# cgtuebingen/3D-RE-GEN

Measured on AMD Instinct MI355X. Metric: objects/sec (50-step Hunyuan3D-2 DiT + 256^3 marching cubes), higher is better.
Workload: dtype bf16; 1 GPU; configs[1]: 5 synthetic 512x512 RGBA crops per GPU, Hunyuan3D-2 full dims bf16, 50 flow-matching steps x CFG 2, 257^3 grid query + Lewiner marching cubes; weights=seeded synthetic, objects_total=5, objects_per_launch=4, parallelism=object-parallel x1

## Files before the change

3d-re-gen_amd/csrc/gemm.hip:

```cpp
#include <hip/hip_runtime.h>
#include <stdint.h>
#include <string.h>

#include <map>
#include <mutex>
#include <type_traits>
#include <utility>

#include "gemm_common.h"
#include "wave_sum.h"
#include "kernels.h"
#include "prof.h"

namespace r3g {
namespace {

constexpr int BK = 64;

template <int B, int E, int S, typename F>
__device__ __forceinline__ void static_for(F&& f) {
    if constexpr (B < E) {
        f(std::integral_constant<int, B>{});
        static_for<B + S, E, S>(f);
    }
}

template <bool GLDS, int NW, int ROWS>
__device__ __forceinline__ void stage_tile(const uint16_t* __restrict__ src, int64_t ld, int row0, int rows_valid,
                                           int k0, char* lds_tile, int wid, int lane, int tid) {
    if constexpr (GLDS) {
#pragma unroll
        for (int i = 0; i < ROWS / 8 / NW; ++i) {
            const int piece = wid * (ROWS / 8 / NW) + i;
            const int row = piece * 8 + (lane >> 3);
            const int kc = (lane & 7) ^ ((row >> 1) & 7);
            int gr = row0 + row;
            gr = gr < rows_valid ? gr : rows_valid - 1;
            const uint16_t* g = src + (int64_t)gr * ld + k0 + kc * 8;
            __builtin_amdgcn_global_load_lds((const __attribute__((address_space(1))) void*)g,
                                             (__attribute__((address_space(3))) void*)(lds_tile + piece * 1024), 16, 0, 0);
        }
    } else {
        uint4 v[ROWS / 8 / NW];
#pragma unroll
        for (int i = 0; i < ROWS / 8 / NW; ++i) {
            const int c = i * (NW * 64) + tid;
            const int row = c >> 3, kc = c & 7;
            int gr = row0 + row;
            gr = gr < rows_valid ? gr : rows_valid - 1;
            v[i] = *reinterpret_cast<const uint4*>(src + (int64_t)gr * ld + k0 + kc * 8);
        }
#pragma unroll
        for (int i = 0; i < ROWS / 8 / NW; ++i) {
            const int c = i * (NW * 64) + tid;
            const int row = c >> 3, kc = c & 7;
            *reinterpret_cast<uint4*>(lds_tile + row * 128 + ((kc ^ ((row >> 1) & 7)) << 4)) = v[i];
        }
    }
}

#define R3G_LDS __attribute__((address_space(3)))
typedef R3G_LDS char* LdsP;
typedef uint32_t u32x4v __attribute__((ext_vector_type(4)));
typedef uint32_t u32x2v __attribute__((ext_vector_type(2)));
__device__ __forceinline__ uint4 lds_ld4(const R3G_LDS char* a) { const u32x4v v = *reinterpret_cast<const R3G_LDS u32x4v*>(a); return make_uint4(v[0], v[1], v[2], v[3]); }
__device__ __forceinline__ uint2 lds_ld2(const R3G_LDS char* a) { const u32x2v v = *reinterpret_cast<const R3G_LDS u32x2v*>(a); return make_uint2(v[0], v[1]); }
__device__ __forceinline__ void lds_st2(R3G_LDS char* a, uint2 v) { *reinterpret_cast<R3G_LDS u32x2v*>(a) = (u32x2v){v.x, v.y}; }
__device__ __forceinline__ LdsP lds_ptr(char* generic_smem_ptr) { return (LdsP)generic_smem_ptr; }

template <int EPI, int MI, bool SMALLREG, int PI = MI, bool VM0 = false, int SLICE = 2048>
__device__ __forceinline__ void gemm_epilogue(const GemmArgs& p, f32x4 (&acc)[4][MI], int m0, int n0, int batch, int wr,
                                              int wc, int lane, LdsP lds_wave = nullptr, bool have_lds = false,
                                              const f32x4* bias_pre = nullptr) {
    constexpr int WROWS = MI * 16;
    static_assert(MI % PI == 0, "scratch passes");
    static_assert(SLICE == 2048 || ((EPI == EPI_QKV || EPI == EPI_BF16 || EPI == EPI_BF16_GELU_TANH || EPI == EPI_BF16_GELU_ERF || EPI == EPI_BF16_GELU_ERF_LNF) && PI == 4),
                  "sliced scratch: 64-row passes of 128-byte rows");
    auto roff = [](int R) __attribute__((always_inline)) { return SLICE == 2048 ? R * 128 : (R >> 4) * SLICE + (R & 15) * 128; };
    if constexpr (EPI == EPI_QKV) {
        const QkvEpi& e = p.qkv;
        const int g = (n0 + wc * 64) >> 6;
        if (n0 + wc * 64 >= p.N) {
            if (VM0) asm volatile("s_waitcnt vmcnt(0)" ::: "memory");
            return;
        }
        int type, head;
        if (e.layout == QKV_KHD) { type = g / e.heads; head = g - type * e.heads; }
        else if (e.layout == QKV_HEAD_QKV) { head = g / 3; type = g - head * 3; }
        else if (e.layout == QKV_HEAD_KV) { head = g >> 1; type = 1 + (g & 1); }
        else { type = 0; head = g; }
        const int dbase = (lane >> 4) << 2;
        int sg_n = e.nseg, sg_m0[3], sg_m1[3], sg_b[3], sg_d[3];
#pragma unroll
        for (int sgi = 0; sgi < 3; ++sgi) { sg_m0[sgi] = e.seg_m0[sgi]; sg_m1[sgi] = e.seg_m1[sgi]; sg_b[sgi] = e.seg_batch[sgi]; sg_d[sgi] = e.seg_dst[sgi]; }
        if (e.nseg > 3) {
            const int mw_u = __builtin_amdgcn_readfirstlane(m0 + wr * WROWS);
            const int4* tab = reinterpret_cast<const int4*>(e.seg_tab);
            int4 t = make_int4(0, 0, 0, 0);
            if (lane < e.nseg) t = tab[lane];
            const int first = __popcll(__ballot(lane < e.nseg && t.y <= mw_u));
            sg_n = 3;
#pragma unroll
            for (int sgi = 0; sgi < 3; ++sgi) {
                const int idx = first + sgi;
                const bool ok = idx < e.nseg;
                const int li = ok ? idx : 0;
                sg_m0[sgi] = ok ? __builtin_amdgcn_readlane(t.x, li) : 0;
                sg_m1[sgi] = ok ? __builtin_amdgcn_readlane(t.y, li) : 0;
                sg_b[sgi] = __builtin_amdgcn_readlane(t.z, li);
                sg_d[sgi] = __builtin_amdgcn_readlane(t.w, li);
            }
        }
        const float* nw = type == 0 ? e.qw : e.kw;
        const float* nb = type == 0 ? e.qb : e.kb;
        const bool do_norm = type < 2 && e.norm != QKN_NONE;
        f32x4 bias4[4], nw4[4], nb4[4];
#pragma unroll
        for (int j = 0; j < 4; ++j) {
            bias4[j] = (f32x4){0.f, 0.f, 0.f, 0.f};
            nw4[j] = (f32x4){1.f, 1.f, 1.f, 1.f};
            nb4[j] = (f32x4){0.f, 0.f, 0.f, 0.f};
            if (p.bias) bias4[j] = *reinterpret_cast<const f32x4*>(p.bias + n0 + wc * 64 + j * 16 + dbase);
            if (do_norm && nw) nw4[j] = *reinterpret_cast<const f32x4*>(nw + j * 16 + dbase);
            if (do_norm && e.norm == QKN_LAYERNORM && nb) nb4[j] = *reinterpret_cast<const f32x4*>(nb + j * 16 + dbase);
        }
        constexpr int PROWS = PI * 16;
        auto flush_pass = [&](const int ip) __attribute__((always_inline)) {
            __builtin_amdgcn_fence(__ATOMIC_ACQ_REL, "wavefront");
            __builtin_amdgcn_wave_barrier();
            if (VM0 && ip == 0) asm volatile("s_waitcnt vmcnt(0)" ::: "memory");
            auto map_row = [&](int m, int& ob, int64_t& drow) {
                ob = batch;
                drow = (int64_t)e.dst_row0 + m;
                if (m >= p.M) return false;
                if (sg_n == 0) return true;
                bool hit = false;
#pragma unroll
                for (int sgi = 0; sgi < 3; ++sgi)
                    if (sgi < sg_n && m >= sg_m0[sgi] && m < sg_m1[sgi]) {
                        hit = true;
                        ob = sg_b[sgi];
                        drow = (int64_t)sg_d[sgi] + (m - sg_m0[sgi]);
                    }
                return hit;
            };
            const int mw = m0 + wr * WROWS + ip * 16;
            const int mw_u = __builtin_amdgcn_readfirstlane(mw);
            bool whole = mw_u + PROWS <= p.M;
            int w_ob = batch;
            int64_t w_drow = (int64_t)e.dst_row0 + mw_u;
            if (sg_n > 0) {
                bool hit = false;
#pragma unroll
                for (int sgi = 0; sgi < 3; ++sgi)
                    if (sgi < sg_n && mw_u >= sg_m0[sgi] && mw_u + PROWS <= sg_m1[sgi]) {
                        hit = true;
                        w_ob = sg_b[sgi];
                        w_drow = (int64_t)sg_d[sgi] + (mw_u - sg_m0[sgi]);
                    }
                whole = whole && hit;
// ... 165 lines not shown
            }
            if (type < 2) {
                uint16_t* base = (type == 0 ? e.Q + (((int64_t)ob * e.heads + head) * e.Lq_pad + drow) * 64
                                            : e.K + (((int64_t)ob * e.heads + head) * e.Lk_pad + drow) * 64);
#pragma unroll
                for (int j = 0; j < 4; ++j) {
                    uint2 pk;
                    pk.x = pack_bf16(v[j][0], v[j][1]);
                    pk.y = pack_bf16(v[j][2], v[j][3]);
                    *reinterpret_cast<uint2*>(base + j * 16 + dbase) = pk;
                }
            } else {
                uint16_t* base = e.Vt + (((int64_t)ob * e.heads + head) * 64) * (int64_t)e.Lk_pad + vt_key_pos(drow);
#pragma unroll
                for (int j = 0; j < 4; ++j)
#pragma unroll
                    for (int c = 0; c < 4; ++c)
                        base[(int64_t)(j * 16 + dbase + c) * e.Lk_pad] = (uint16_t)(pack_bf16(v[j][c], 0.f) & 0xFFFFu);
            }
        }
        if constexpr (kWide) flush_pass(ip);
        });
        };
        if (have_lds) all_passes(std::true_type{});
        else all_passes(std::false_type{});
        return;
    }
    const int mrow = m0 + wr * WROWS + (lane & 15);
    const int ncol = n0 + wc * 64 + ((lane >> 4) << 2);
    const float* gate = p.gate ? p.gate + (int64_t)batch * p.strideGate : nullptr;
    if constexpr (EPI == EPI_FP8_GELU_ERF) {
        uint8_t* C8 = reinterpret_cast<uint8_t*>(p.C) + (int64_t)batch * p.strideC;
        const float inv = p.out_inv_scale;
        const bool wide = have_lds && PI == MI && (p.N & 15) == 0 && (p.ldc & 15) == 0 && (p.strideC & 15) == 0 &&
                          (reinterpret_cast<uintptr_t>(p.C) & 15) == 0;
#pragma unroll
        for (int j = 0; j < 4; ++j) {
            const int n = ncol + j * 16;
            f32x4 bj = (f32x4){0.f, 0.f, 0.f, 0.f};
            if (p.bias) bj = *reinterpret_cast<const f32x4*>(p.bias + (n < p.N ? n : p.N - 4));
#pragma unroll
            for (int i = 0; i < MI; ++i) {
                f32x4 v = gelu_erf4<false>(acc[j][i] + bj) * inv;
#pragma unroll
                for (int c = 0; c < 4; ++c) v[c] = __builtin_fabsf(v[c]) > 448.f ? __builtin_copysignf(448.f, v[c]) : v[c];
                int w = 0;
                w = __builtin_amdgcn_cvt_pk_fp8_f32(v[0], v[1], w, false);
                w = __builtin_amdgcn_cvt_pk_fp8_f32(v[2], v[3], w, true);
                const int r = i * 16 + (lane & 15), m = mrow + i * 16;
                if (wide) *reinterpret_cast<R3G_LDS uint32_t*>(lds_wave + r * 64 + ((j ^ (r & 3)) << 4) + ((lane >> 4) << 2)) = (uint32_t)w;
                else if (n < p.N && m < p.M) *reinterpret_cast<uint32_t*>(C8 + (int64_t)m * p.ldc + n) = (uint32_t)w;
            }
        }
        if (wide) {
            __builtin_amdgcn_fence(__ATOMIC_ACQ_REL, "wavefront");
            __builtin_amdgcn_wave_barrier();
            const int cc = lane & 3, n = n0 + wc * 64 + cc * 16;
#pragma unroll
            for (int t = 0; t < WROWS / 16; ++t) {
                const int rr = t * 16 + (lane >> 2);
                const int m = m0 + wr * WROWS + rr;
                const uint4 d = lds_ld4(lds_wave + rr * 64 + ((cc ^ (rr & 3)) << 4));
                if (m < p.M && n < p.N) *reinterpret_cast<uint4*>(C8 + (int64_t)m * p.ldc + n) = d;
            }
        }
        return;
    }
    if constexpr (EPI == EPI_RESID_BF16 || EPI == EPI_RESID_F16 || EPI == EPI_RESID_BF16_LND || EPI == EPI_RESID_BF16_ST) {
        constexpr bool F16 = EPI == EPI_RESID_F16;
        constexpr bool ST = EPI == EPI_RESID_BF16_ST;
        constexpr bool LND = EPI == EPI_RESID_BF16_LND || ST;
        uint16_t* X = reinterpret_cast<uint16_t*>(p.C) + (int64_t)batch * p.strideC;
        const uint16_t* XR = p.resid_src ? p.resid_src + (int64_t)batch * p.strideC : X;
        f32x4 bj[4], gj[4];
#pragma unroll
        for (int j = 0; j < 4; ++j) {
            const int nb = ncol + j * 16;
            const int nbc = nb < p.N ? nb : p.N - 4;
            bj[j] = (f32x4){0.f, 0.f, 0.f, 0.f};
            gj[j] = (f32x4){1.f, 1.f, 1.f, 1.f};
            if (p.bias) bj[j] = *reinterpret_cast<const f32x4*>(p.bias + nbc);
            if (gate) gj[j] = *reinterpret_cast<const f32x4*>(gate + nbc);
        }
        const bool wide = have_lds && PI >= 2 && (p.N & 7) == 0 && (p.ldc & 7) == 0 && (p.strideC & 7) == 0 &&
                          (reinterpret_cast<uintptr_t>(p.C) & 15) == 0 && (reinterpret_cast<uintptr_t>(XR) & 15) == 0;
        if (wide) {
            constexpr int RP = PI * 8;
            constexpr int GP = PI / 2;
            const int cc = lane & 7;
            const int n = n0 + wc * 64 + cc * 8;
            f32x4 gw0 = (f32x4){0.f, 0.f, 0.f, 0.f}, gw1 = gw0;
            if constexpr (LND && !ST) {
                const int nc = n < p.N ? n : p.N - 8;
                gw0 = *reinterpret_cast<const f32x4*>(p.lnd_gw + nc);
                gw1 = *reinterpret_cast<const f32x4*>(p.lnd_gw + nc + 4);
            }
            const bool full = m0 + wr * WROWS + WROWS <= p.M && n0 + wc * 64 + 64 <= p.N;
            const int64_t row0 = (int64_t)(m0 + wr * WROWS + (lane >> 3)) * p.ldc + n, step8 = 8 * (int64_t)p.ldc;
#pragma unroll
            for (int ip = 0; ip < MI; ip += GP) {
                uint4 old[RP / 8];
                if (full) {
#pragma unroll
                    for (int t = 0; t < RP / 8; ++t)
                        old[t] = *reinterpret_cast<const uint4*>(XR + row0 + (int64_t)(ip * 2 + t) * step8);
                } else {
#pragma unroll
                    for (int t = 0; t < RP / 8; ++t) {
                        const int m = m0 + wr * WROWS + ip * 16 + t * 8 + (lane >> 3);
                        const int mc = m < p.M ? m : p.M - 1;
                        const int nc = n < p.N ? n : p.N - 8;
                        old[t] = *reinterpret_cast<const uint4*>(XR + (int64_t)mc * p.ldc + nc);
                    }
                }
#pragma unroll
                for (int j = 0; j < 4; ++j)
#pragma unroll
                    for (int ii = 0; ii < GP; ++ii) {
                        const int r = ii * 16 + (lane & 15);
                        const int chunk = (j * 4 + (lane >> 4)) ^ (r & 15);
                        *reinterpret_cast<R3G_LDS f32x4*>(lds_wave + r * 256 + chunk * 16) = gj[j] * (acc[j][ip + ii] + bj[j]);
                    }
                __builtin_amdgcn_fence(__ATOMIC_ACQ_REL, "wavefront");
                __builtin_amdgcn_wave_barrier();
                auto rows_out = [&](auto FULLC) __attribute__((always_inline)) {
                constexpr bool kFull = decltype(FULLC)::value;
#pragma unroll
                for (int t = 0; t < RP / 8; ++t) {
                    const int rr = t * 8 + (lane >> 3);
                    const int m = m0 + wr * WROWS + ip * 16 + rr;
                    const f32x4 d0 = *reinterpret_cast<const R3G_LDS f32x4*>(lds_wave + rr * 256 + (((2 * cc) ^ (rr & 15)) << 4));
                    const f32x4 d1 = *reinterpret_cast<const R3G_LDS f32x4*>(lds_wave + rr * 256 + (((2 * cc + 1) ^ (rr & 15)) << 4));
                    const uint32_t o[4] = {old[t].x, old[t].y, old[t].z, old[t].w};
                    uint32_t q[4];
#pragma unroll
                    for (int k = 0; k < 4; ++k) {
                        const f32x2 ov = unpack16<F16>(o[k]);
                        const f32x4& d = k < 2 ? d0 : d1;
                        q[k] = pack16<F16>(ov[0] + d[(k & 1) * 2], ov[1] + d[(k & 1) * 2 + 1]);
                    }
                    if constexpr (LND) {
                        float v[8];
#pragma unroll
                        for (int k = 0; k < 4; ++k) {
                            const f32x2 u = unpack16<false>(q[k]);
                            v[2 * k] = u[0];
                            v[2 * k + 1] = u[1];
                        }
                        float s1 = ((v[0] + v[1]) + (v[2] + v[3])) + ((v[4] + v[5]) + (v[6] + v[7]));
                        s1 += lane_xor<1>(s1);
                        s1 += lane_xor<2>(s1);
                        s1 += lane_xor<4>(s1);
                        const float mu = s1 * (1.0f / 64.0f);
                        float m2 = 0.f, s3 = 0.f;
#pragma unroll
                        for (int k = 0; k < 8; ++k) {
                            const float dv = v[k] - mu;
                            m2 = fmaf(dv, dv, m2);
                            s3 = fmaf(v[k], k < 4 ? gw0[k] : gw1[k - 4], s3);
                        }
                        m2 += lane_xor<1>(m2); s3 += lane_xor<1>(s3);
                        m2 += lane_xor<2>(m2); s3 += lane_xor<2>(s3);
                        m2 += lane_xor<4>(m2); s3 += lane_xor<4>(s3);
                        if (cc == 0 && m < p.M && n < p.N)
                            *reinterpret_cast<f32x4*>(p.lnd_part + ((int64_t)m * (p.N >> 6) + ((n0 >> 6) + wc)) * 4) = (f32x4){s1, m2, s3, 0.f};
                    }
                    if constexpr (!LND || ST) {
                        if constexpr (kFull) *reinterpret_cast<uint4*>(X + row0 + (int64_t)(ip * 2 + t) * step8) = make_uint4(q[0], q[1], q[2], q[3]);
                        else if (m < p.M && n < p.N) *reinterpret_cast<uint4*>(X + (int64_t)m * p.ldc + n) = make_uint4(q[0], q[1], q[2], q[3]);
                    }
                }
                };
                if (full) rows_out(std::true_type{});
                else rows_out(std::false_type{});
                __builtin_amdgcn_fence(__ATOMIC_ACQ_REL, "wavefront");
                __builtin_amdgcn_wave_barrier();
            }
            return;
        }
        if constexpr (LND) return;
#pragma unroll
        for (int j = 0; j < 4; ++j) {
            uint2 old[MI];
#pragma unroll
            for (int i = 0; i < MI; ++i) {
                const int n = ncol + j * 16, m = mrow + i * 16;
                const int nc = n < p.N ? n : p.N - 4, mc = m < p.M ? m : p.M - 1;
                old[i] = *reinterpret_cast<const uint2*>(XR + (int64_t)mc * p.ldc + nc);
            }
#pragma unroll
            for (int i = 0; i < MI; ++i) {
                const int n = ncol + j * 16, m = mrow + i * 16;
                const f32x4 d = gj[j] * (acc[j][i] + bj[j]);
                uint2 pk;
                const f32x2 ox = unpack16<F16>(old[i].x), oy = unpack16<F16>(old[i].y);
                pk.x = pack16<F16>(ox[0] + d[0], ox[1] + d[1]);
                pk.y = pack16<F16>(oy[0] + d[2], oy[1] + d[3]);
                if (n < p.N && m < p.M) *reinterpret_cast<uint2*>(X + (int64_t)m * p.ldc + n) = pk;
            }
        }
        return;
    }
    if constexpr (EPI == EPI_RESID_F32) {
        float* X = reinterpret_cast<float*>(p.C) + (int64_t)batch * p.strideC;
        const bool wide = have_lds && (p.ldc & 3) == 0 && (p.strideC & 3) == 0 &&
                          (reinterpret_cast<uintptr_t>(p.C) & 15) == 0;
        if (wide) {
            const int cc = lane & 7;
#pragma unroll
            for (int jp = 0; jp < 2; ++jp) {
                f32x4 bj[2], gj[2];
#pragma unroll
                for (int jj = 0; jj < 2; ++jj) {
                    const int nb = ncol + (2 * jp + jj) * 16;
                    const int nbc = nb < p.N ? nb : p.N - 4;
                    bj[jj] = (f32x4){0.f, 0.f, 0.f, 0.f};
                    gj[jj] = (f32x4){1.f, 1.f, 1.f, 1.f};
                    if (p.bias) bj[jj] = *reinterpret_cast<const f32x4*>(p.bias + nbc);
                    if (gate) gj[jj] = *reinterpret_cast<const f32x4*>(gate + nbc);
                }
                const int n = n0 + wc * 64 + jp * 32 + cc * 4;
                const int nc = n < p.N ? n : p.N - 4;
#pragma unroll
                for (int ip = 0; ip < MI; ip += PI) {
#pragma unroll
                    for (int jj = 0; jj < 2; ++jj)
#pragma unroll
                        for (int ii = 0; ii < PI; ++ii) {
                            const int r = ii * 16 + (lane & 15);
                            const int chunk = (jj * 4 + (lane >> 4)) ^ (r & 7);
                            *reinterpret_cast<R3G_LDS f32x4*>(lds_wave + r * 128 + chunk * 16) = gj[jj] * (acc[2 * jp + jj][ip + ii] + bj[jj]);
                        }
                    __builtin_amdgcn_fence(__ATOMIC_ACQ_REL, "wavefront");
                    __builtin_amdgcn_wave_barrier();
                    if (VM0 && jp == 0 && ip == 0) asm volatile("s_waitcnt vmcnt(0)" ::: "memory");
#pragma unroll
                    for (int t0 = 0; t0 < PI * 2; t0 += 4) {
                        f32x4 old[4];
#pragma unroll
                        for (int tt = 0; tt < 4; ++tt) {
                            const int m = m0 + wr * WROWS + ip * 16 + (t0 + tt) * 8 + (lane >> 3);
                            const int mc = m < p.M ? m : p.M - 1;
                            old[tt] = *reinterpret_cast<const f32x4*>(X + (int64_t)mc * p.ldc + nc);
                        }
#pragma unroll
                        for (int tt = 0; tt < 4; ++tt) {
                            const int rr = (t0 + tt) * 8 + (lane >> 3);
                            const int m = m0 + wr * WROWS + ip * 16 + rr;
                            const f32x4 d = *reinterpret_cast<const R3G_LDS f32x4*>(lds_wave + rr * 128 + ((cc ^ (rr & 7)) << 4));
                            if (n < p.N && m < p.M) *reinterpret_cast<f32x4*>(X + (int64_t)m * p.ldc + n) = old[tt] + d;
                        }
                    }
                    __builtin_amdgcn_fence(__ATOMIC_ACQ_REL, "wavefront");
// ... 1109 lines not shown
        R3G_SB();
        R3G_BAR();
        read_a(1, b);
        R3G_SB();
        if (!last) stage_a(0, t + 2, b);
        R3G_BAR();
        R3G_SB();
        mma(I1{}, I1{});
        R3G_SB();
        R3G_BAR();
        if (!last) {
            stage_w(1, t + 2, b);
            asm volatile("s_waitcnt vmcnt(6)" ::: "memory");
        } else if (b == 0) {
            asm volatile("s_waitcnt vmcnt(0)" ::: "memory");
        }
        R3G_BAR();
        R3G_SB();
        mma(I1{}, I0{});
        R3G_SB();
        R3G_BAR();
    };
    using T = std::true_type;
    using F = std::false_type;

    auto locate_u = [&](int index, Tile& tl, int& nk) {
        tl = locate(index);
        tl.second = __builtin_amdgcn_readfirstlane(tl.second);
        tl.batch = __builtin_amdgcn_readfirstlane(tl.batch);
        tl.m0 = __builtin_amdgcn_readfirstlane(tl.m0);
        tl.n0 = __builtin_amdgcn_readfirstlane(tl.n0);
        nk = args_of(tl.second).K / BK;
    };
    Tile cur;
    int nk;
    int my = wg_first;
    locate_u(my, cur, nk);
    set_sources(cur);
    stage_w(0, 0, 0); stage_a(0, 0, 0); stage_w(1, 0, 0); stage_a(1, 0, 0);
    R3G_STAMP_DECL;
    for (;;) {
        R3G_STAMP(5);
        stage_w(0, 1, 1); stage_a(0, 1, 1); stage_w(1, 1, 1);
        __builtin_amdgcn_s_waitcnt(0x0F76);
        R3G_BAR();
        if (wr == 1) R3G_BAR();
        R3G_STAMP(0);
        int t = 0;
        for (; t + 2 < nk; t += 2) {
            four_phases(I0{}, F{}, t);
            four_phases(I1{}, F{}, t + 1);
        }
        four_phases(I0{}, T{}, t);
        four_phases(I1{}, T{}, t + 1);
        if (wr == 0) R3G_BAR();
        R3G_STAMP(1);

        const Tile done = cur;
        int lane_e = lane;
        asm volatile("" : "+v"(lane_e));
        f32x4 bias_pre[4];
        {
            const GemmArgs& pp = args_of(done.second);
#pragma unroll
            for (int j = 0; j < 4; ++j) {
                const int n = done.n0 + wc * 64 + ((lane_e >> 4) << 2) + j * 16;
                bias_pre[j] = (f32x4){0.f, 0.f, 0.f, 0.f};
                if (pp.bias) bias_pre[j] = *reinterpret_cast<const f32x4*>(pp.bias + (n < pp.N ? n : pp.N - 4));
            }
        }
        my += xcd_wgs;
        const bool more = my < xcd_end;
        if (more) {
            locate_u(my, cur, nk);
            set_sources(cur);
            stage_w(0, 0, 0); stage_a(0, 0, 0); stage_w(1, 0, 0); stage_a(1, 0, 0);
        }
        R3G_STAMP(2);
        {
            const GemmArgs& pp = args_of(done.second);
            auto run = [&](auto E) __attribute__((always_inline)) {
                constexpr int epi = decltype(E)::value;
                constexpr bool kPre = epi == EPI_BF16 || epi == EPI_BF16_GELU_TANH || epi == EPI_BF16_GELU_ERF || epi == EPI_BF16_GELU_ERF_LNF;
                constexpr bool kSl = SLICED && (kPre || epi == EPI_QKV);
                if constexpr (kSl)
                    gemm_epilogue<epi, MI, true, 4, false, HALF>(pp, acc, done.m0, done.n0, done.batch, wr, wc, lane_e,
                                                                 lds_ptr(smem + BUF + wid * 2048), true, kPre ? bias_pre : nullptr);
                else
                    gemm_epilogue<epi, MI, true, 2, false>(pp, acc, done.m0, done.n0, done.batch, wr, wc, lane_e,
                                                           lds_ptr(smem + 2 * BUF + wid * 4096), pp.wide_epilogue != 0, kPre ? bias_pre : nullptr);
            };
            if constexpr (EPI2 != EPI) {
                if (done.second) run(std::integral_constant<int, EPI2>{});
                else run(std::integral_constant<int, EPI>{});
            } else {
                run(std::integral_constant<int, EPI>{});
            }
        }
        R3G_STAMP(3);
        if (!more) break;
        asm volatile("" : "+s"(cur.m0), "+s"(cur.n0), "+s"(cur.batch));
        set_sources(cur);
#pragma unroll
        for (int j = 0; j < 4; ++j)
#pragma unroll
            for (int i = 0; i < MI; ++i) acc[j][i] = (f32x4){0.f, 0.f, 0.f, 0.f};
    }
    R3G_STAMP_OUT;
}

#ifdef R3G_GEMM_STAMPS
}
}
extern "C" __attribute__((visibility("default"))) int r3g_debug_gemm_stamps(unsigned long long* out64) {
    return (int)hipMemcpyFromSymbol(out64, HIP_SYMBOL(r3g::g_gemm_stamps), sizeof(unsigned long long) * 64);
}
namespace r3g {
namespace {
#endif

int g_gemm_xcd_walk = 1;
int g_gemm_persistent_qkv = 1;
int g_gemm_epi_slices = 1;
int g_gemm_mixed = 1;

template <int EPI, int EPI2 = EPI>
hipError_t launch_gemm8p(const GemmArgs& p, const GemmArgs& p2, int num_cu, hipStream_t s) {
    int tiles = ((p.N + 255) / 256) * ((p.M + 255) / 256) * p.batch;
    if (p2.M > 0) tiles += ((p2.N + 255) / 256) * ((p2.M + 255) / 256) * p2.batch;
    const int rounds = (tiles + num_cu - 1) / num_cu;
    const int grid = (tiles + rounds - 1) / rounds;
    const size_t lds = 163840;
    constexpr bool kSliceable = EPI == EPI_BF16 || EPI == EPI_BF16_GELU_TANH || EPI == EPI_BF16_GELU_ERF || EPI == EPI_QKV || EPI == EPI_BF16_GELU_ERF_LNF;
    auto k = gemm8p_kernel<EPI, false, EPI2>;
    auto ks = gemm8p_kernel<EPI, kSliceable, EPI2>;
    static int state = 0;
    if (state == 0) {
        state = hipFuncSetAttribute((const void*)k, hipFuncAttributeMaxDynamicSharedMemorySize, (int)lds) == hipSuccess ? 1 : -1;
        if (state > 0 && kSliceable)
            state = hipFuncSetAttribute((const void*)ks, hipFuncAttributeMaxDynamicSharedMemorySize, (int)lds) == hipSuccess ? 1 : -1;
    }
    if (state < 0) { (void)hipGetLastError(); return hipErrorNotSupported; }
    const int walk = g_gemm_xcd_walk ? rounds : 0;
    counter_add(EPI2 != EPI ? LC_GEMM_MIXED : LC_GEMM_PHASED_PERSISTENT);
    if (kSliceable && g_gemm_epi_slices && p.wide_epilogue) { hipLaunchKernelGGL(ks, dim3(grid), dim3(512), lds, s, p, p2, tiles, walk); }
    else { hipLaunchKernelGGL(k, dim3(grid), dim3(512), lds, s, p, p2, tiles, walk); }
    return hipGetLastError();
}

template <int EPI>
hipError_t launch_gemm8(const GemmArgs& p, const GemmArgs& p2, hipStream_t s) {
    int tiles = ((p.N + 255) / 256) * ((p.M + 255) / 256) * p.batch;
    if (p2.M > 0) tiles += ((p2.N + 255) / 256) * ((p2.M + 255) / 256) * p2.batch;
    const size_t lds = 131072;
    auto k = gemm8_kernel<EPI, false>;
    static bool done = false;
    if (!done) {
        done = true;
        (void)hipFuncSetAttribute((const void*)k, hipFuncAttributeMaxDynamicSharedMemorySize, (int)lds);
    }
    counter_add(LC_GEMM_PHASED);
    hipLaunchKernelGGL(k, dim3(tiles), dim3(512), lds, s, p, p2, (float*)nullptr, (unsigned*)nullptr, 0u);
    return hipGetLastError();
}

constexpr int kSplitMaxTiles = 128;
struct SplitWs { float* ws = nullptr; unsigned* flags = nullptr; unsigned epoch = 0; };
static std::mutex g_split_mutex;
static std::map<std::pair<int, hipStream_t>, SplitWs> g_split;

template <int EPI>
hipError_t launch_gemm8_split(const GemmArgs& p, const GemmArgs& p2, hipStream_t s) {
    int tiles = ((p.N + 255) / 256) * ((p.M + 255) / 256) * p.batch;
    if (p2.M > 0) tiles += ((p2.N + 255) / 256) * ((p2.M + 255) / 256) * p2.batch;
    if (tiles > kSplitMaxTiles) return hipErrorNotSupported;
    int dev = 0;
    hipError_t e = hipGetDevice(&dev);
    if (e != hipSuccess) return e;
    SplitWs w;
    {
        std::lock_guard<std::mutex> lock(g_split_mutex);
        SplitWs& slot = g_split[std::make_pair(dev, s)];
        if (!slot.ws) {
            e = hipMalloc((void**)&slot.ws, (size_t)kSplitMaxTiles * 256 * 256 * 4);
            if (e != hipSuccess) return e;
            e = hipMalloc((void**)&slot.flags, (size_t)kSplitMaxTiles * 8 * 4);
            if (e != hipSuccess) return e;
            e = hipMemset(slot.flags, 0, (size_t)kSplitMaxTiles * 8 * 4);
            if (e != hipSuccess) return e;
        }
        if (++slot.epoch == 0u) slot.epoch = 1u;
        w = slot;
    }
    const size_t lds = 131072;
    auto k = gemm8_kernel<EPI, true>;
    static bool done = false;
    if (!done) {
        done = true;
        (void)hipFuncSetAttribute((const void*)k, hipFuncAttributeMaxDynamicSharedMemorySize, (int)lds);
    }
    counter_add(LC_GEMM_SPLITK2);
    hipLaunchKernelGGL(k, dim3(2 * tiles), dim3(512), lds, s, p, p2, w.ws, w.flags, w.epoch);
    return hipGetLastError();
}

template <int EPI>
hipError_t launch_deep(const GemmArgs& p, int batch, hipStream_t s) {
    const int tiles = ((p.N + 255) / 256) * ((p.M + 255) / 256) * batch;
    const size_t lds = 4 * 2 * 256 * 32 * 2;
    auto k = gemm_deep_kernel<EPI>;
    static bool done = false;
    if (!done) {
        done = true;
        (void)hipFuncSetAttribute((const void*)k, hipFuncAttributeMaxDynamicSharedMemorySize, (int)lds);
    }
    counter_add(LC_GEMM_DEEP_RING);
// ... 14 lines not shown
        if (!done) {
            done = true;
            (void)hipFuncSetAttribute((const void*)kt, hipFuncAttributeMaxDynamicSharedMemorySize, (int)lds);
            (void)hipFuncSetAttribute((const void*)kf, hipFuncAttributeMaxDynamicSharedMemorySize, (int)lds);
        }
    }
    counter_add(BIG == 2 ? LC_GEMM_256X128 : BIG == 1 ? (NW == 16 ? LC_GEMM_W16_256 : LC_GEMM_TWO_STAGE_256) : (NW == 4 ? LC_GEMM_W4_128 : LC_GEMM_W8_128));
    if (!glds) counter_add(LC_GEMM_REGISTER_STAGED);
    if (glds) {
        hipLaunchKernelGGL(kt, dim3(tiles), dim3(NW * 64), lds, s, p, p2);
    } else {
        hipLaunchKernelGGL(kf, dim3(tiles), dim3(NW * 64), lds, s, p, p2);
    }
    return hipGetLastError();
}

template <bool RESID>
__global__ __launch_bounds__(256) void splitk_reduce_kernel(const float* __restrict__ ws, int S, int64_t MN, int N,
                                                            const float* __restrict__ bias, const float* __restrict__ gate,
                                                            float* __restrict__ C, int64_t ldc) {
    const int64_t i = ((int64_t)blockIdx.x * 256 + threadIdx.x) * 4;
    if (i >= MN) return;
    f32x4 v = *reinterpret_cast<const f32x4*>(ws + i);
    int s = 1;
    for (; s + 4 <= S; s += 4) {
        f32x4 t[4];
#pragma unroll
        for (int k = 0; k < 4; ++k) t[k] = *reinterpret_cast<const f32x4*>(ws + (int64_t)(s + k) * MN + i);
#pragma unroll
        for (int k = 0; k < 4; ++k) v += t[k];
    }
    for (; s < S; ++s) v += *reinterpret_cast<const f32x4*>(ws + (int64_t)s * MN + i);
    const int64_t m = i / N;
    const int n = (int)(i - m * N);
    if (bias) v += *reinterpret_cast<const f32x4*>(bias + n);
    float* dst = C + m * ldc + n;
    if (RESID) {
        if (gate) v = *reinterpret_cast<const f32x4*>(gate + n) * v;
        v = *reinterpret_cast<const f32x4*>(dst) + v;
    }
    *reinterpret_cast<f32x4*>(dst) = v;
}

int g_gemm_splitk128 = 1;
constexpr int kSplit128Slots = 512;
constexpr int kSplit128MinSteps = 8;

static int splitk128_factor(int M, int N, int K, int num_cu) {
    if (K < 2048 || K % 64) return 1;
    const long tiles = (long)((M + 127) / 128) * ((N + 127) / 128);
    const long slots = (long)kSplit128Slots * num_cu / 256;
    if (tiles * 2 > slots) return 1;
    const int nk = K / 64;
    int best = 1;
    for (int S = 2; S <= 64 && S * tiles <= slots && nk / S >= kSplit128MinSteps; ++S)
        if (nk % S == 0) best = S;
    if (best == 2 && K < 4096) best = 1;
    return best;
}

int g_conv_implicit = 1;

template <int EPI>
hipError_t launch_conv(const GemmArgs& p, hipStream_t s) {
    const int tiles = ((p.N + 127) / 128) * ((p.M + 127) / 128) * p.batch;
    const size_t lds = (size_t)2 * (128 + 128) * BK * 2;
    auto k = conv_gemm_kernel<EPI>;
    static bool done = false;
    if (!done) {
        done = true;
        (void)hipFuncSetAttribute((const void*)k, hipFuncAttributeMaxDynamicSharedMemorySize, (int)lds);
    }
    counter_add(LC_GEMM_CONV_IMPLICIT);
    hipLaunchKernelGGL(k, dim3(tiles), dim3(512), lds, s, p);
    return hipGetLastError();
}

int g_gemm_waves = 0;
int g_gemm_raster = -1;
int g_gemm_auto_rule = 2;
int g_num_cu = 256;
int g_gemm_splitk = 0;
int g_gemm_persistent_resid = 0;
int g_gemm_persistent = 1;
int g_gemm_phased = 1;
int g_gemm_wide_epilogue = 1;
int g_gemm_gelu_pk = 1;

template <int EPI>
hipError_t launch_epi(const GemmArgs& p, const GemmArgs& p2, bool glds, hipStream_t s) {
    int waves = g_gemm_waves;
    const int batch = p.batch;
    if (waves == 0) {
        long t256 = (long)((p.N + 255) / 256) * ((p.M + 255) / 256) * batch;
        if (p2.M > 0) t256 += (long)((p2.N + 255) / 256) * ((p2.M + 255) / 256) * p2.batch;
        const long rounds = (t256 + g_num_cu - 1) / g_num_cu;
        const bool fills = t256 * 10 >= rounds * g_num_cu * 9;
        if (g_gemm_auto_rule == 0) {
            if (p2.M == 0 && p.N % 256 == 0 && t256 >= 128 && (p.K >= 2048 || t256 >= 2048)) waves = 9;
            else waves = p.N <= 1024 ? 8 : 4;
        } else {
            const bool wide_enough = p.N >= 4096 || (g_gemm_auto_rule >= 2 && t256 * 100 >= (long)g_num_cu * 85);
            if ((p2.M == 0 || p2.N % 256 == 0) && p.N % 256 == 0 && t256 >= 128 &&
                (p.K >= 2048 || t256 >= 2048 || (wide_enough && fills)))
                waves = g_gemm_phased ? 11 : 9;
            else waves = 8;
        }
    }
    if constexpr (EPI == EPI_RESID_F32 || EPI == EPI_RESID_BF16 || EPI == EPI_RESID_F16 || EPI == EPI_BF16) {
        long tiles = (long)((p.N + 255) / 256) * ((p.M + 255) / 256) * p.batch;
        if (p2.M > 0) tiles += (long)((p2.N + 255) / 256) * ((p2.M + 255) / 256) * p2.batch;
        const bool shape_ok = p.K % 256 == 0 && p.K >= 512 && (p2.M == 0 || p2.K == p.K) && p.N % 256 == 0 &&
                              (p2.M == 0 || p2.N % 256 == 0) && 2 * tiles <= g_num_cu && tiles <= kSplitMaxTiles;
        if (shape_ok && (waves == 13 || (g_gemm_splitk && g_gemm_waves == 0 && EPI == EPI_RESID_F32 && p.K >= 2048 &&
                                         2 * tiles > g_num_cu / 2))) {
            const hipError_t e = launch_gemm8_split<EPI>(p, p2, s);
            if (e != hipErrorNotSupported) return e;
        }
        if (waves == 13) waves = 11;
    }
    if (waves == 13) waves = 11;
    if ((waves == 11 || waves == 12) && p.K % 128 == 0 && (p2.M == 0 || p2.K % 128 == 0)) {
        {
            long tiles = (long)((p.N + 255) / 256) * ((p.M + 255) / 256) * p.batch;
            if (p2.M > 0) tiles += (long)((p2.N + 255) / 256) * ((p2.M + 255) / 256) * p2.batch;
            const bool resid_ok = (EPI != EPI_RESID_F32 || (g_gemm_persistent_resid & 1)) &&
                                  ((EPI != EPI_RESID_BF16 && EPI != EPI_RESID_F16) || (g_gemm_persistent_resid & 2)) &&
                                  (EPI != EPI_QKV || (g_gemm_persistent_qkv && p.wide_epilogue));
            if (p.K >= 256 && (p2.M == 0 || p2.K >= 256) &&
                (waves == 12 || (g_gemm_persistent && g_gemm_waves == 0 && tiles > g_num_cu && resid_ok && EPI != EPI_F32))) {
                const hipError_t e = launch_gemm8p<EPI>(p, p2, g_num_cu, s);
                if (e != hipErrorNotSupported) return e;
            }
        }
        return launch_gemm8<EPI>(p, p2, s);
    }
    if (waves == 11 || waves == 12) waves = g_gemm_waves == 0 ? 9 : 8;
    if (waves == 32 && p.K % 32 == 0 && p2.M == 0) return launch_deep<EPI>(p, batch, s);
    if (waves == 16) return launch_cfg<EPI, 16, 1>(p, p2, glds, s);
    if (waves == 9) return launch_cfg<EPI, 8, 1>(p, p2, glds, s);
    if (waves == 10) return launch_cfg<EPI, 8, 2>(p, p2, glds, s);
    if (waves == 8) return launch_cfg<EPI, 8, 0>(p, p2, glds, s);
    return launch_cfg<EPI, 4, 0>(p, p2, glds, s);
}

}

int g_gemm_glds = 1;

const Option g_gemm_options[] = {
    {"gemm_waves", &g_gemm_waves, OPT_KEEP,
     [](int v) { return v == 0 || v == 4 || v == 8 || v == 9 || v == 10 || v == 11 || v == 12 || v == 13 || v == 16 || v == 32; }},
    {"gemm_raster", &g_gemm_raster, OPT_ANY},
    {"gemm_auto_rule", &g_gemm_auto_rule, OPT_KEEP, [](int v) { return v >= 0; }},
    {"gemm_num_cu", &g_num_cu, OPT_KEEP, [](int v) { return v > 0; }},
    {"gemm_wide_epilogue", &g_gemm_wide_epilogue},
    {"gemm_phased", &g_gemm_phased},
    {"gemm_persistent", &g_gemm_persistent},
    {"gemm_persistent_resid", &g_gemm_persistent_resid, OPT_MASK, nullptr, 3},
    {"gemm_splitk", &g_gemm_splitk},
    {"gemm_splitk128", &g_gemm_splitk128},
    {"conv_implicit", &g_conv_implicit},
    {"gemm_xcd_walk", &g_gemm_xcd_walk},
    {"gemm_epi_slices", &g_gemm_epi_slices},
    {"gemm_mixed", &g_gemm_mixed},
    {"gemm_persistent_qkv", &g_gemm_persistent_qkv},
    {"gelu_pk", &g_gemm_gelu_pk},
    {}};

bool gemm_conv_implicit() { return g_conv_implicit && g_gemm_glds && g_gemm_waves == 0; }
bool gemm_auto_takes_256(int M, int N, int K) {
    if (g_gemm_waves != 0 || g_gemm_auto_rule == 0) return false;
    const long t256 = (long)((N + 255) / 256) * ((M + 255) / 256);
    const long rounds = (t256 + g_num_cu - 1) / g_num_cu;
    const bool fills = t256 * 10 >= rounds * g_num_cu * 9;
    const bool wide_enough = N >= 4096 || (g_gemm_auto_rule >= 2 && t256 * 100 >= (long)g_num_cu * 85);
    return N % 256 == 0 && t256 >= 128 && (K >= 2048 || t256 >= 2048 || (wide_enough && fills));
}
int gemm_splitk128_factor(int M, int N, int K) { return splitk128_factor(M, N, K, g_num_cu); }

bool gemm_fold_supported(int epi, int M, int N, int K) {
    if (epi != EPI_RESID_BF16_ST && epi != EPI_BF16_GELU_ERF_LNF && epi != EPI_RESID_BF16_LND) return false;
    if (!g_gemm_glds || !g_gemm_wide_epilogue) return false;
    return M > 0 && N > 0 && K % 128 == 0 && K >= 256 && N % 256 == 0;
}

static bool gemm_args_ok(const GemmArgs& p) {
    if (p.epi == EPI_QKV && p.qkv.nseg > 3) {
        if (p.qkv.nseg > 64) return false;
        const int* t = p.qkv.seg_tab_host;
        if (!t || !p.qkv.seg_tab) return false;
        for (int i = 0; i < p.qkv.nseg; ++i) {
            if (t[4 * i] > t[4 * i + 1]) return false;
            if (i > 0 && t[4 * i] < t[4 * (i - 1) + 1]) return false;
            if (i >= 3 && t[4 * i] - t[4 * (i - 3) + 1] + 1 < 128) return false;
        }
    }
    return !(p.K % 64 != 0 || p.K <= 0 || (p.N & 3) || (p.lda & 7) || (p.ldw & 7) || (p.epi == EPI_QKV && p.N % 64));
}

static int g_last_splitk_slices = 1;
int gemm_last_splitk_slices() { return g_last_splitk_slices; }

hipError_t gemm_launch2(const GemmArgs& p_in, int batch, const GemmArgs* p2_in, int batch2, hipStream_t s) {
    GemmArgs p = p_in, p2{};
    g_last_splitk_slices = 1;
    p.batch = batch;
    p.raster_group = g_gemm_raster;
    p.wide_epilogue = g_gemm_wide_epilogue ? 1 : 0;
    p.gelu_pk = g_gemm_gelu_pk ? 1 : 0;
    if (p2_in && p2_in->M > 0 && p2_in->N > 0 && batch2 > 0) {
        p2 = *p2_in;
        p2.batch = batch2;
        p2.raster_group = p.raster_group;
        p2.wide_epilogue = p.wide_epilogue;
        p2.gelu_pk = p.gelu_pk;
        if (p2.epi != p.epi || !gemm_args_ok(p2)) return hipErrorInvalidValue;
    }
    if (p.M <= 0 || p.N <= 0 || batch <= 0) {
        if (p2.M > 0) return gemm_launch2(*p2_in, batch2, nullptr, 0, s);
        return hipSuccess;
    }
    if (!gemm_args_ok(p)) return hipErrorInvalidValue;
    auto alg_bytes = [](const GemmArgs& g) {
        if (g.M <= 0) return 0.0;
        const double out = g.epi == EPI_RESID_F32 ? 8.0 : (g.epi == EPI_F32 || g.epi == EPI_RESID_BF16 || g.epi == EPI_RESID_F16 ? 4.0 : g.epi == EPI_RESID_BF16_LND ? 2.0 : (g.epi == EPI_FP8_GELU_ERF ? 1.0 : 2.0));
        return (double)g.batch * (2.0 * g.M * g.K + out * (double)g.M * g.N) + 2.0 * (double)g.N * g.K;
    };
    ProfScope ps(PC_GEMM, 2.0 * (double)p.M * p.N * p.K * batch + 2.0 * (double)p2.M * p2.N * p2.K * p2.batch, s,
                 alg_bytes(p) + alg_bytes(p2));
    if (p.conv.x) {
        const ConvA& cv = p.conv;
        if (p2.M > 0 || batch != 1 || (p.epi != EPI_F32 && p.epi != EPI_RESID_F32) || !g_gemm_glds || cv.Cin < 64 || cv.Cin % 64 ||
            p.K != 9 * cv.Cin || !cv.zero || cv.Ho < 1 || cv.Wo < 1 || p.M % (cv.Ho * cv.Wo) || (p.ldc & 3) ||
            (reinterpret_cast<uintptr_t>(p.C) & 15))
            return hipErrorInvalidValue;
        const int64_t MN = (int64_t)p.M * p.N;
        int S = 1;
        if (p.split_ws && g_gemm_splitk128) {
            S = splitk128_factor(p.M, p.N, p.K, g_num_cu);
            if ((int64_t)S * MN > p.split_ws_elems) S = 1;
        }
        if (S > 1) {
            g_last_splitk_slices = S;
            counter_add(LC_GEMM_SPLITK128);
            GemmArgs q = p;
            q.K = p.K / S;
            q.batch = S;
            q.strideW = q.K;
            q.bias = nullptr;
            q.gate = nullptr;
            q.C = p.split_ws;
            q.ldc = p.N;
            q.strideC = MN;
            q.epi = EPI_F32;
            q.split_ws = nullptr;
            const hipError_t e = launch_conv<EPI_F32>(q, s);
            if (e != hipSuccess) return e;
            const unsigned blocks = (unsigned)((MN / 4 + 255) / 256);
            if (p.epi == EPI_RESID_F32)
                hipLaunchKernelGGL(splitk_reduce_kernel<true>, dim3(blocks), dim3(256), 0, s, (const float*)p.split_ws, S, MN, p.N,
                                   p.bias, p.gate, reinterpret_cast<float*>(p.C), p.ldc);
            else
                hipLaunchKernelGGL(splitk_reduce_kernel<false>, dim3(blocks), dim3(256), 0, s, (const float*)p.split_ws, S, MN, p.N,
                                   p.bias, p.gate, reinterpret_cast<float*>(p.C), p.ldc);
            return hipGetLastError();
        }
        return p.epi == EPI_F32 ? launch_conv<EPI_F32>(p, s) : launch_conv<EPI_RESID_F32>(p, s);
    }
    if (p.split_ws && g_gemm_splitk128 && g_gemm_waves == 0 && p2.M == 0 && batch == 1 && (p.epi == EPI_F32 || p.epi == EPI_RESID_F32) &&
        (p.ldc & 3) == 0 && (reinterpret_cast<uintptr_t>(p.C) & 15) == 0) {
        const int S = splitk128_factor(p.M, p.N, p.K, g_num_cu);
        const int64_t MN = (int64_t)p.M * p.N;
        if (S > 1 && (int64_t)S * MN <= p.split_ws_elems) {
            g_last_splitk_slices = S;
            counter_add(LC_GEMM_SPLITK128);
            GemmArgs q = p;
            q.K = p.K / S;
            q.batch = S;
            q.strideA = q.K;
            q.strideW = q.K;
            q.bias = nullptr;
            q.gate = nullptr;
            q.C = p.split_ws;
            q.ldc = p.N;
            q.strideC = MN;
            q.epi = EPI_F32;
            q.split_ws = nullptr;
            const hipError_t e = launch_cfg<EPI_F32, 8, 0>(q, GemmArgs{}, g_gemm_glds, s);
            if (e != hipSuccess) return e;
            const unsigned blocks = (unsigned)((MN / 4 + 255) / 256);
            if (p.epi == EPI_RESID_F32)
                hipLaunchKernelGGL(splitk_reduce_kernel<true>, dim3(blocks), dim3(256), 0, s, (const float*)p.split_ws, S, MN, p.N,
                                   p.bias, p.gate, reinterpret_cast<float*>(p.C), p.ldc);
            else
                hipLaunchKernelGGL(splitk_reduce_kernel<false>, dim3(blocks), dim3(256), 0, s, (const float*)p.split_ws, S, MN, p.N,
                                   p.bias, p.gate, reinterpret_cast<float*>(p.C), p.ldc);
            return hipGetLastError();
        }
    }
    if (p.epi == EPI_RESID_BF16_ST) {
        const uint16_t* xr = p.resid_src ? p.resid_src : reinterpret_cast<const uint16_t*>(p.C);
        if (p2.M > 0 || batch != 1 || !g_gemm_glds || !p.wide_epilogue || !p.lnd_part || p.K % 128 || p.K < 256 || p.N % 256 || (p.ldc & 7) ||
            (reinterpret_cast<uintptr_t>(p.C) & 15) || (reinterpret_cast<uintptr_t>(xr) & 15) || (reinterpret_cast<uintptr_t>(p.lnd_part) & 15))
            return hipErrorInvalidValue;
        return launch_gemm8<EPI_RESID_BF16_ST>(p, p2, s);
    }
    if (p.epi == EPI_BF16_GELU_ERF_LNF) {
        const long tiles = (long)(p.N / 256) * ((p.M + 255) / 256);
        if (p2.M > 0 || batch != 1 || !g_gemm_glds || !p.wide_epilogue || !p.lnf_c1 || !p.lnf_stats || !p.bias || p.K % 128 || p.K < 256 ||
            p.N % 256 || (p.ldc & 7) || (reinterpret_cast<uintptr_t>(p.C) & 15) || tiles < 1)
            return hipErrorInvalidValue;
        return launch_gemm8p<EPI_BF16_GELU_ERF_LNF>(p, p2, g_num_cu, s);
    }
    if (p.epi == EPI_RESID_BF16_LND) {
        const uint16_t* xr = p.resid_src ? p.resid_src : reinterpret_cast<const uint16_t*>(p.C);
        if (p2.M > 0 || batch != 1 || !g_gemm_glds || !p.wide_epilogue || !p.lnd_gw || !p.lnd_part || p.gate || p.K % 128 || p.K < 256 ||
            p.N % 256 || (p.ldc & 7) || (reinterpret_cast<uintptr_t>(p.C) & 15) || (reinterpret_cast<uintptr_t>(xr) & 15) ||
            (reinterpret_cast<uintptr_t>(p.lnd_gw) & 15) || (reinterpret_cast<uintptr_t>(p.lnd_part) & 15))
            return hipErrorInvalidValue;
        return launch_gemm8<EPI_RESID_BF16_LND>(p, p2, s);
    }
    switch (p.epi) {
        case EPI_BF16: return launch_epi<EPI_BF16>(p, p2, g_gemm_glds, s);
        case EPI_BF16_GELU_TANH: return launch_epi<EPI_BF16_GELU_TANH>(p, p2, g_gemm_glds, s);
        case EPI_BF16_GELU_ERF: return launch_epi<EPI_BF16_GELU_ERF>(p, p2, g_gemm_glds, s);
        case EPI_RESID_F32: return launch_epi<EPI_RESID_F32>(p, p2, g_gemm_glds, s);
        case EPI_F32: return launch_epi<EPI_F32>(p, p2, g_gemm_glds, s);
        case EPI_QKV: return launch_epi<EPI_QKV>(p, p2, g_gemm_glds, s);
        case EPI_RESID_BF16: return launch_epi<EPI_RESID_BF16>(p, p2, g_gemm_glds, s);
        case EPI_RESID_F16: return launch_epi<EPI_RESID_F16>(p, p2, g_gemm_glds, s);
        default: return hipErrorInvalidValue;
    }
}

hipError_t gemm_launch(const GemmArgs& p, int batch, hipStream_t s) { return gemm_launch2(p, batch, nullptr, 0, s); }

hipError_t gemm_launch_qkv_mlp(const GemmArgs& pq_in, const GemmArgs& pm_in, hipStream_t s) {
    GemmArgs pq = pq_in, pm = pm_in;
    auto fallback = [&]() {
        const hipError_t e = gemm_launch(pm_in, 1, s);
        return e != hipSuccess ? e : gemm_launch(pq_in, 1, s);
    };
    if (!g_gemm_mixed || !g_gemm_persistent || !g_gemm_persistent_qkv || !g_gemm_phased || g_gemm_waves != 0 || !g_gemm_glds || !g_gemm_wide_epilogue ||
        pq.epi != EPI_QKV || pm.epi != EPI_BF16_GELU_TANH || pq.conv.x || pm.conv.x || pq.M <= 0 || pm.M <= 0)
        return fallback();
    if (pq.K % 128 || pm.K % 128 || pq.K < 256 || pm.K < 256 || pq.N % 256 || pm.N % 256) return fallback();
    const long tiles = (long)(pq.N / 256) * ((pq.M + 255) / 256) + (long)(pm.N / 256) * ((pm.M + 255) / 256);
    const long rounds = (tiles + g_num_cu - 1) / g_num_cu;
    if (tiles < 2L * g_num_cu || tiles * 10 < rounds * g_num_cu * 9) return fallback();
    for (GemmArgs* g : {&pq, &pm}) {
        g->batch = 1;
        g->raster_group = g_gemm_raster;
        g->wide_epilogue = 1;
        g->gelu_pk = g_gemm_gelu_pk ? 1 : 0;
        if (!gemm_args_ok(*g)) return hipErrorInvalidValue;
    }
    auto alg_bytes = [](const GemmArgs& g) { return 2.0 * g.M * g.K + 2.0 * (double)g.M * g.N + 2.0 * (double)g.N * g.K; };
    ProfScope ps(PC_GEMM, 2.0 * (double)pq.M * pq.N * pq.K + 2.0 * (double)pm.M * pm.N * pm.K, s, alg_bytes(pq) + alg_bytes(pm));
    const hipError_t e = launch_gemm8p<EPI_QKV, EPI_BF16_GELU_TANH>(pq, pm, g_num_cu, s);
    if (e == hipErrorNotSupported) return fallback();
    return e;
}

hipError_t gemm_fp8_launch(const GemmArgs& p_in, const float* scale_a, const float* scale_w, hipStream_t s) {
    GemmArgs p = p_in;
    if (p.M < 0 || p.N < 0) return hipErrorInvalidValue;
    if (p.M == 0 || p.N == 0) return hipSuccess;
    if (p.K % 256 || p.K < 256 || (p.lda & 15) || (p.ldw & 15) || (p.N & 3) || !scale_a || !scale_w) return hipErrorInvalidValue;
    if ((int64_t)p.M * p.lda >= (1ll << 32) || (int64_t)p.N * p.ldw >= (1ll << 32)) return hipErrorInvalidValue;
    p.batch = 1;
    p.K /= 2; p.lda /= 2; p.ldw /= 2;
    p.raster_group = g_gemm_raster;
    p.wide_epilogue = g_gemm_wide_epilogue ? 1 : 0;
    ProfScope ps(PC_GEMM, 2.0 * (double)p.M * p.N * (2.0 * p.K), s);
    switch (p.epi) {
        case EPI_BF16: return launch_gemm8_fp8<EPI_BF16>(p, scale_a, scale_w, s);
        case EPI_BF16_GELU_TANH: return launch_gemm8_fp8<EPI_BF16_GELU_TANH>(p, scale_a, scale_w, s);
        case EPI_BF16_GELU_ERF: return launch_gemm8_fp8<EPI_BF16_GELU_ERF>(p, scale_a, scale_w, s);
        case EPI_RESID_F32: return launch_gemm8_fp8<EPI_RESID_F32>(p, scale_a, scale_w, s);
        case EPI_RESID_BF16: return launch_gemm8_fp8<EPI_RESID_BF16>(p, scale_a, scale_w, s);
        case EPI_QKV: return launch_gemm8_fp8<EPI_QKV>(p, scale_a, scale_w, s);
        case EPI_FP8_GELU_ERF: return launch_gemm8_fp8<EPI_FP8_GELU_ERF>(p, scale_a, scale_w, s);
        default: return hipErrorInvalidValue;
    }
}

}
```

Before: 0.8246 objects/sec.

## Route 16-bit residual GEMM epilogues through persistent sliced-scratch kernel by default

Extends the sliced LDS scratch layout (32 rows of 256 bytes) to the 16-bit residual epilogues so they can run in the persistent 8-wave kernel with overlapped epilogue. Enables the persistent path by default for residual-stats and LND residual GEMMs, and for plain bf16/f16 residual GEMMs with K>=1024 and at most two waves of tiles, via a compile-time auto mask. The epilogue also batches LDS reads ahead of the stores and drops the gate multiply in the LND case. The aim is to cut non-persistent launch tail and epilogue stalls, at the cost of more code paths and different tile scheduling.

```diff
diff --git a/3d-re-gen_amd/csrc/gemm.hip b/3d-re-gen_amd/csrc/gemm.hip
--- a/3d-re-gen_amd/csrc/gemm.hip
+++ b/3d-re-gen_amd/csrc/gemm.hip
@@ -74,8 +74,9 @@
                                               const f32x4* bias_pre = nullptr) {
     constexpr int WROWS = MI * 16;
     static_assert(MI % PI == 0, "scratch passes");
-    static_assert(SLICE == 2048 || ((EPI == EPI_QKV || EPI == EPI_BF16 || EPI == EPI_BF16_GELU_TANH || EPI == EPI_BF16_GELU_ERF || EPI == EPI_BF16_GELU_ERF_LNF) && PI == 4),
-                  "sliced scratch: 64-row passes of 128-byte rows");
+    static_assert(SLICE == 2048 || ((EPI == EPI_QKV || EPI == EPI_BF16 || EPI == EPI_BF16_GELU_TANH || EPI == EPI_BF16_GELU_ERF || EPI == EPI_BF16_GELU_ERF_LNF ||
+                                     EPI == EPI_RESID_F16 || EPI == EPI_RESID_BF16 || EPI == EPI_RESID_BF16_ST || EPI == EPI_RESID_BF16_LND) && PI == 4),
+                  "sliced scratch: 64-row passes of 128-byte rows (the 16-bit residual epilogues: 32 rows of 256 bytes)");
     auto roff = [](int R) __attribute__((always_inline)) { return SLICE == 2048 ? R * 128 : (R >> 4) * SLICE + (R & 15) * 128; };
     if constexpr (EPI == EPI_QKV) {
         const QkvEpi& e = p.qkv;
@@ -407,11 +408,13 @@
             if (p.bias) bj[j] = *reinterpret_cast<const f32x4*>(p.bias + nbc);
             if (gate) gj[j] = *reinterpret_cast<const f32x4*>(gate + nbc);
         }
+        constexpr bool kNoGate = LND && !ST && SLICE != 2048;
         const bool wide = have_lds && PI >= 2 && (p.N & 7) == 0 && (p.ldc & 7) == 0 && (p.strideC & 7) == 0 &&
                           (reinterpret_cast<uintptr_t>(p.C) & 15) == 0 && (reinterpret_cast<uintptr_t>(XR) & 15) == 0;
         if (wide) {
             constexpr int RP = PI * 8;
             constexpr int GP = PI / 2;
+            auto roff256 = [](int R) __attribute__((always_inline)) { return SLICE == 2048 ? R * 256 : (R >> 3) * SLICE + (R & 7) * 256; };
             const int cc = lane & 7;
             const int n = n0 + wc * 64 + cc * 8;
             f32x4 gw0 = (f32x4){0.f, 0.f, 0.f, 0.f}, gw1 = gw0;
@@ -444,18 +447,39 @@
                     for (int ii = 0; ii < GP; ++ii) {
                         const int r = ii * 16 + (lane & 15);
                         const int chunk = (j * 4 + (lane >> 4)) ^ (r & 15);
-                        *reinterpret_cast<R3G_LDS f32x4*>(lds_wave + r * 256 + chunk * 16) = gj[j] * (acc[j][ip + ii] + bj[j]);
+                        if constexpr (kNoGate) *reinterpret_cast<R3G_LDS f32x4*>(lds_wave + roff256(r) + chunk * 16) = acc[j][ip + ii] + bj[j];
+                        else *reinterpret_cast<R3G_LDS f32x4*>(lds_wave + roff256(r) + chunk * 16) = gj[j] * (acc[j][ip + ii] + bj[j]);
                     }
                 __builtin_amdgcn_fence(__ATOMIC_ACQ_REL, "wavefront");
                 __builtin_amdgcn_wave_barrier();
                 auto rows_out = [&](auto FULLC) __attribute__((always_inline)) {
                 constexpr bool kFull = decltype(FULLC)::value;
-#pragma unroll
-                for (int t = 0; t < RP / 8; ++t) {
+                constexpr bool kReadFirst = SLICE != 2048;
+                constexpr int RA = kReadFirst && LND ? 2 : RP / 8;
+#pragma unroll
+                for (int tg = 0; tg < RP / 8; tg += RA) {
+                f32x4 dd[kReadFirst ? RA : 1][2];
+                if constexpr (kReadFirst) {
+#pragma unroll
+                    for (int tt = 0; tt < RA; ++tt) {
+                        const int rr = (tg + tt) * 8 + (lane >> 3);
+                        dd[tt][0] = *reinterpret_cast<const R3G_LDS f32x4*>(lds_wave + roff256(rr) + (((2 * cc) ^ (rr & 15)) << 4));
+                        dd[tt][1] = *reinterpret_cast<const R3G_LDS f32x4*>(lds_wave + roff256(rr) + (((2 * cc + 1) ^ (rr & 15)) << 4));
+                    }
+                    __builtin_amdgcn_sched_barrier(0);
+                }
+#pragma unroll
+                for (int t = tg; t < tg + RA; ++t) {
                     const int rr = t * 8 + (lane >> 3);
                     const int m = m0 + wr * WROWS + ip * 16 + rr;
-                    const f32x4 d0 = *reinterpret_cast<const R3G_LDS f32x4*>(lds_wave + rr * 256 + (((2 * cc) ^ (rr & 15)) << 4));
-                    const f32x4 d1 = *reinterpret_cast<const R3G_LDS f32x4*>(lds_wave + rr * 256 + (((2 * cc + 1) ^ (rr & 15)) << 4));
+                    f32x4 d0, d1;
+                    if constexpr (kReadFirst) {
+                        d0 = dd[t - tg][0];
+                        d1 = dd[t - tg][1];
+                    } else {
+                        d0 = *reinterpret_cast<const R3G_LDS f32x4*>(lds_wave + rr * 256 + (((2 * cc) ^ (rr & 15)) << 4));
+                        d1 = *reinterpret_cast<const R3G_LDS f32x4*>(lds_wave + rr * 256 + (((2 * cc + 1) ^ (rr & 15)) << 4));
+                    }
                     const uint32_t o[4] = {old[t].x, old[t].y, old[t].z, old[t].w};
                     uint32_t q[4];
 #pragma unroll
@@ -494,6 +518,7 @@
                         if constexpr (kFull) *reinterpret_cast<uint4*>(X + row0 + (int64_t)(ip * 2 + t) * step8) = make_uint4(q[0], q[1], q[2], q[3]);
                         else if (m < p.M && n < p.N) *reinterpret_cast<uint4*>(X + (int64_t)m * p.ldc + n) = make_uint4(q[0], q[1], q[2], q[3]);
                     }
+                }
                 }
                 };
                 if (full) rows_out(std::true_type{});
@@ -1769,7 +1794,8 @@
             auto run = [&](auto E) __attribute__((always_inline)) {
                 constexpr int epi = decltype(E)::value;
                 constexpr bool kPre = epi == EPI_BF16 || epi == EPI_BF16_GELU_TANH || epi == EPI_BF16_GELU_ERF || epi == EPI_BF16_GELU_ERF_LNF;
-                constexpr bool kSl = SLICED && (kPre || epi == EPI_QKV);
+                constexpr bool kRmw16 = epi == EPI_RESID_F16 || epi == EPI_RESID_BF16 || epi == EPI_RESID_BF16_ST || epi == EPI_RESID_BF16_LND;
+                constexpr bool kSl = SLICED && (kPre || epi == EPI_QKV || kRmw16);
                 if constexpr (kSl)
                     gemm_epilogue<epi, MI, true, 4, false, HALF>(pp, acc, done.m0, done.n0, done.batch, wr, wc, lane_e,
                                                                  lds_ptr(smem + BUF + wid * 2048), true, kPre ? bias_pre : nullptr);
@@ -1818,7 +1844,8 @@
     const int rounds = (tiles + num_cu - 1) / num_cu;
     const int grid = (tiles + rounds - 1) / rounds;
     const size_t lds = 163840;
-    constexpr bool kSliceable = EPI == EPI_BF16 || EPI == EPI_BF16_GELU_TANH || EPI == EPI_BF16_GELU_ERF || EPI == EPI_QKV || EPI == EPI_BF16_GELU_ERF_LNF;
+    constexpr bool kSliceable = EPI == EPI_BF16 || EPI == EPI_BF16_GELU_TANH || EPI == EPI_BF16_GELU_ERF || EPI == EPI_QKV || EPI == EPI_BF16_GELU_ERF_LNF ||
+                                EPI == EPI_RESID_F16 || EPI == EPI_RESID_BF16 || EPI == EPI_RESID_BF16_ST || EPI == EPI_RESID_BF16_LND;
     auto k = gemm8p_kernel<EPI, false, EPI2>;
     auto ks = gemm8p_kernel<EPI, kSliceable, EPI2>;
     static int state = 0;
@@ -1999,6 +2026,9 @@
 int g_num_cu = 256;
 int g_gemm_splitk = 0;
 int g_gemm_persistent_resid = 0;
+#ifndef R3G_GEMM_RESID_AUTO
+#define R3G_GEMM_RESID_AUTO 7
+#endif
 int g_gemm_persistent = 1;
 int g_gemm_phased = 1;
 int g_gemm_wide_epilogue = 1;
@@ -2041,8 +2071,9 @@
         {
             long tiles = (long)((p.N + 255) / 256) * ((p.M + 255) / 256) * p.batch;
             if (p2.M > 0) tiles += (long)((p2.N + 255) / 256) * ((p2.M + 255) / 256) * p2.batch;
+            const bool resid16_auto = tiles <= 2L * g_num_cu && p2.M == 0 && p.K >= 1024 && (R3G_GEMM_RESID_AUTO & 4);
             const bool resid_ok = (EPI != EPI_RESID_F32 || (g_gemm_persistent_resid & 1)) &&
-                                  ((EPI != EPI_RESID_BF16 && EPI != EPI_RESID_F16) || (g_gemm_persistent_resid & 2)) &&
+                                  ((EPI != EPI_RESID_BF16 && EPI != EPI_RESID_F16) || (g_gemm_persistent_resid & 2) || resid16_auto) &&
                                   (EPI != EPI_QKV || (g_gemm_persistent_qkv && p.wide_epilogue));
             if (p.K >= 256 && (p2.M == 0 || p2.K >= 256) &&
                 (waves == 12 || (g_gemm_persistent && g_gemm_waves == 0 && tiles > g_num_cu && resid_ok && EPI != EPI_F32))) {
@@ -2100,6 +2131,11 @@
     if (epi != EPI_RESID_BF16_ST && epi != EPI_BF16_GELU_ERF_LNF && epi != EPI_RESID_BF16_LND) return false;
     if (!g_gemm_glds || !g_gemm_wide_epilogue) return false;
     return M > 0 && N > 0 && K % 128 == 0 && K >= 256 && N % 256 == 0;
+}
+
+static bool resid_stats_persistent(const GemmArgs& p, int cls) {
+    const long tiles = (long)(p.N / 256) * ((p.M + 255) / 256);
+    return g_gemm_persistent && tiles > g_num_cu && ((g_gemm_persistent_resid & 2) || (R3G_GEMM_RESID_AUTO & cls));
 }
 
 static bool gemm_args_ok(const GemmArgs& p) {
@@ -2221,6 +2257,10 @@
         if (p2.M > 0 || batch != 1 || !g_gemm_glds || !p.wide_epilogue || !p.lnd_part || p.K % 128 || p.K < 256 || p.N % 256 || (p.ldc & 7) ||
             (reinterpret_cast<uintptr_t>(p.C) & 15) || (reinterpret_cast<uintptr_t>(xr) & 15) || (reinterpret_cast<uintptr_t>(p.lnd_part) & 15))
             return hipErrorInvalidValue;
+        if (resid_stats_persistent(p, 1)) {
+            const hipError_t e = launch_gemm8p<EPI_RESID_BF16_ST>(p, p2, g_num_cu, s);
+            if (e != hipErrorNotSupported) return e;
+        }
         return launch_gemm8<EPI_RESID_BF16_ST>(p, p2, s);
     }
     if (p.epi == EPI_BF16_GELU_ERF_LNF) {
@@ -2236,6 +2276,10 @@
             p.N % 256 || (p.ldc & 7) || (reinterpret_cast<uintptr_t>(p.C) & 15) || (reinterpret_cast<uintptr_t>(xr) & 15) ||
             (reinterpret_cast<uintptr_t>(p.lnd_gw) & 15) || (reinterpret_cast<uintptr_t>(p.lnd_part) & 15))
             return hipErrorInvalidValue;
+        if (resid_stats_persistent(p, 2)) {
+            const hipError_t e = launch_gemm8p<EPI_RESID_BF16_LND>(p, p2, g_num_cu, s);
+            if (e != hipErrorNotSupported) return e;
+        }
         return launch_gemm8<EPI_RESID_BF16_LND>(p, p2, s);
     }
     switch (p.epi) {
```

After: 0.8301 objects/sec (median of 6 runs). No clear change (+0.7%).
